# andres-fr/realtime-pose-estimation

Hardware: AMD Instinct MI355X
Metric: images/sec at 640x640 (HRNet-w48 fwd+decode) (higher is better)
Workload: dtype f16 (fp32 accumulate, fp32 BatchNorm; fp32 NCHW in/out); 1 GPU; configs[2]: batch=32 per GPU, 640x640, half-wrapper teacher forward + decode of 17 keypoint channels, weights W0 (seeded random); batch_per_gpu=32, people_per_batch_rank0=960

## Files before the change

realtime-pose-estimation_amd/csrc/engine.hip:

```cpp
#include <stdarg.h>

#include <chrono>
#include <mutex>
#include <map>
#include <tuple>
#include <vector>

#include "rtpe_common.h"

namespace rtpe {

static thread_local std::string g_err;

void set_error(const char* fmt, ...) {
  char buf[1024];
  va_list ap;
  va_start(ap, fmt);
  vsnprintf(buf, sizeof(buf), fmt, ap);
  va_end(ap);
  g_err = buf;
}

int hip_fail(hipError_t e, const char* what, const char* file, int line) {
  set_error("HIP error %d (%s) at %s:%d: %s", (int)e, hipGetErrorString(e), file, line, what);
// ... 10 lines not shown
  int fuse;
  int pair;
  int stem2;
  int s2g;
};

}

using namespace rtpe;

struct rtpe_hrnet {
  int device;
  std::vector<OpState> ops;
  std::map<std::tuple<int, int, int>, std::vector<ConvTile>> tuned;
  std::map<int, std::vector<hipEvent_t>> records;
  std::vector<rtpe_tensor_desc> tensors;
  std::vector<char> plane_ok;
  int n_slots;
  char* arena;
  size_t arena_bytes;
  int n_preds, n_refined;
  std::mutex lane_mu;
  hipStream_t lane_stream[4] = {nullptr, nullptr, nullptr, nullptr};
  std::vector<hipEvent_t> op_event;
  std::vector<char> needs_event;
  std::vector<std::vector<int>> wait_ops;
  hipEvent_t fork_event = nullptr;
  bool has_regions = false;
};

static size_t align_up(size_t v, size_t a) { return (v + a - 1) / a * a; }

namespace rtpe {
static int g_options[kNumOptions] = {-1, -1, -1, -1, -1, -1, -1, -1, -1, -1, -1};
static const char* const kOptionNames[kNumOptions] = {"block_ring", "block_pc", "direct_1x1", "lanes", "tile_dma", "pair_1x1", "fused_stem", "conv64", "head_direct", "deconv48", "conv48s2"};
static const char* const kOptionEnv[kNumOptions] = {"RTPE_BLOCK_RING", "RTPE_BLOCK_PC", "RTPE_DIRECT_1X1", "RTPE_LANES", "RTPE_TILE_DMA", "RTPE_PAIR_1X1", "RTPE_FUSED_STEM", "RTPE_CONV64", "RTPE_HEAD_DIRECT", "RTPE_DECONV48", "RTPE_CONV48S2"};
static const int kOptionDefault[kNumOptions] = {0, 1, 1, 1, 1, 1, 1, 1, 1, 1, 1};
int get_option(int key) {
  int v = __atomic_load_n(&g_options[key], __ATOMIC_RELAXED);
  if (v < 0) {
    v = kOptionEnv[key][0] ? env_int(kOptionEnv[key], kOptionDefault[key]) : kOptionDefault[key];
    __atomic_store_n(&g_options[key], v, __ATOMIC_RELAXED);
  }
  return v;
}
}

extern "C" int rtpe_set_option(const char* name, int32_t value) {
  RTPE_REQUIRE(name != nullptr && value >= 0, "set_option: bad argument");
  for (int k = 0; k < kNumOptions; ++k)
    if (kOptionNames[k][0] && strcmp(name, kOptionNames[k]) == 0) {
      __atomic_store_n(&g_options[k], (int)value, __ATOMIC_RELAXED);
      return RTPE_OK;
    }
  set_error("set_option: unknown option '%s'", name);
  return RTPE_E_INVALID;
}

extern "C" int rtpe_get_option(const char* name, int32_t* value) {
  RTPE_REQUIRE(name != nullptr && value != nullptr, "get_option: null argument");
  for (int k = 0; k < kNumOptions; ++k)
    if (kOptionNames[k][0] && strcmp(name, kOptionNames[k]) == 0) {
      *value = get_option(k);
      return RTPE_OK;
    }
  set_error("get_option: unknown option '%s'", name);
  return RTPE_E_INVALID;
}

extern "C" const char* rtpe_last_error_string(void) { return g_err.c_str(); }
// ... 634 lines not shown
        }
        a.N = N; a.H_in = Hi; a.W_in = Wi;
        a.H_full = Ho; a.W_full = Wo;
        if (dc) {
          a.H_pos = Hi; a.W_pos = Wi; a.o_mul = 2; a.oy_add = k >> 1; a.ox_add = k & 1;
        } else {
          a.H_pos = Ho; a.W_pos = Wo; a.o_mul = 1;
        }
        a.relu = (d.flags & RTPE_F_RELU) ? 1 : 0;
        a.round_conv = (d.flags & RTPE_F_ROUND_CONV) ? 1 : 0;
        ConvTile tile;
        if (merge)
          tile = tile0;
        else if (force)
          tile = *force;
        else if (tuned && (*tuned)[i * 4 + k].nt)
          tile = (*tuned)[i * 4 + k];
        else
          tile = conv_make_tile(o.plan[k], N, a.H_pos, a.W_pos);
        const bool direct_ok = a.x_bytes < 0x80000000ull && a.y != nullptr && a.y_nchw == nullptr && a.o_mul == 1;
        if (tile.kind == 4 && !direct_ok) tile = conv_make_tile(o.plan[k], N, a.H_pos, a.W_pos, false);
        if (tile.kind == 5 && !(direct_ok && a.res == nullptr && !plane[d.in_t] && !plane[d.out_t] && get_option(kOptConv64) != 0))
          tile = conv_make_tile(o.plan[k], N, a.H_pos, a.W_pos, true, false);
        conv_fill_args(o.geom[k], o.plan[k], tile, &a);
        if (!merge && force == nullptr && get_option(kOptHeadDirect) != 0 && conv_head_supports(o.plan[k], a)) {
          RTPE_HP_LAUNCH(rc = conv_head_launch(o.plan[k], a, s));
          continue;
        }
        if (!merge && force == nullptr && get_option(kOptConv48s2) != 0 && !plane[d.in_t] && !(a.y != nullptr && plane[d.out_t]) &&
            conv48s2_supports(o.plan[k], a)) {
          RTPE_HP_LAUNCH(rc = conv48s2_launch(o.plan[k], a, s));
          continue;
        }
        if (merge) {
          if (k == 0) { merged = a; merged_tile = tile; merged.n_cls = 4; }
          merged.w_c[k] = a.w;
          merged.lo_yc[k] = a.lo_y; merged.lo_xc[k] = a.lo_x;
          merged.oy_c[k] = a.oy_add; merged.ox_c[k] = a.ox_add;
          if (k == o.n_geom - 1) {
            if (force == nullptr && get_option(kOptDeconv48) != 0 && deconv48_supports(o.plan[0], merged))
              RTPE_HP_LAUNCH(rc = deconv48_launch(o.plan[0], merged, s));
            else
              RTPE_HP_LAUNCH(rc = conv_launch(o.plan[0], merged_tile, merged, s));
          }
          continue;
        }
        if (pairs_on && o.pair == 1 && direct_ok) {
          pair_args = a;
          pair_pending = true;
          continue;
        }
        if (pair_pending) {
          pair_pending = false;
          RTPE_HP_LAUNCH(rc = conv_pair_launch(h->ops[i - 1].plan[0], pair_args, o.plan[0], a, s));
          continue;
        }
        RTPE_HP_LAUNCH(rc = conv_launch(o.plan[k], tile, a, s));
      }
    } else if (d.kind == RTPE_OP_AUX_PACK) {
      if (aux == nullptr) { set_error("forward: this program has a second input (use rtpe_hrnet_forward_aux)"); return RTPE_E_INVALID; }
      const rtpe_tensor_desc& to = h->tensors[d.out_t];
      rc = aux_pack_launch(reinterpret_cast<const float*>(aux), reinterpret_cast<float*>(tptr(d.out_t, d.out_coff)),
                           to.channels, N, H >> to.ds_log2, W >> to.ds_log2, s);
    } else if (d.kind == RTPE_OP_RESIZE) {
      const rtpe_tensor_desc& ti = h->tensors[d.in_t];
      const rtpe_tensor_desc& to = h->tensors[d.out_t];
// ... 178 lines not shown
  char* dev = nullptr;
  const size_t wb = align_up(p.packed_bytes, 256);
  RTPE_HIP_CHECK(hipMalloc(reinterpret_cast<void**>(&dev), wb + ab.size() * 4));
  hipError_t e = hipMemcpy(dev, packed.data(), p.packed_bytes, hipMemcpyHostToDevice);
  if (e == hipSuccess) e = hipMemcpy(dev + wb, ab.data(), ab.size() * 4, hipMemcpyHostToDevice);
  if (e != hipSuccess) { hipFree(dev); return hip_fail(e, "hipMemcpy", __FILE__, __LINE__); }
  ConvArgs a;
  memset(&a, 0, sizeof(a));
  a.x = reinterpret_cast<const _Float16*>(x); a.in_ld = cin;
  a.x_bytes = (size_t)N * H * W * cin * es;
  a.w = reinterpret_cast<const _Float16*>(dev);
  a.alpha = reinterpret_cast<const float*>(dev + wb); a.beta = a.alpha + p.cout_pad;
  a.res = reinterpret_cast<const _Float16*>(res); a.res_ld = cout;
  a.y = reinterpret_cast<_Float16*>(y); a.out_ld = cout; a.cout_store = cout;
  a.N = N; a.H_in = H; a.W_in = W;
  a.H_full = a.H_pos = H / stride; a.W_full = a.W_pos = W / stride; a.o_mul = 1;
  a.relu = (flags & RTPE_F_RELU) ? 1 : 0;
  a.round_conv = (flags & RTPE_F_ROUND_CONV) ? 1 : 0;
  const bool one_window = a.x_bytes < 0x80000000ull;
  const ConvTile tile = conv_make_tile(p, N, a.H_pos, a.W_pos, one_window, one_window && res == nullptr);
  static const int probe_plane = RTPE_DIAG_ENV_INT("RTPE_PROBE_PLANE", 0);
  if (probe_plane && tile.kind == 2 && cin % 48 == 0 && cout % 48 == 0 && stride == 1) {
    a.in_ld = 48; a.in_cs = (long long)N * H * W * 48;
    a.out_ld = 48; a.out_cs = (long long)N * H * W * 48;
    if (res != nullptr) { a.res_ld = 48; a.res_cs = (long long)N * H * W * 48; }
  }
  conv_fill_args(g, p, tile, &a);
#ifdef RTPE_CONV_STAMPS
  unsigned long long* dbg = nullptr;
  hipMalloc(reinterpret_cast<void**>(&dbg), 128);
  hipMemset(dbg, 0, 128);
  a.dbg = dbg;
#endif
  int rc = get_option(kOptConv48s2) != 0 && conv48s2_supports(p, a) ? conv48s2_launch(p, a, s) : conv_launch(p, tile, a, s);
  hipError_t es2 = hipStreamSynchronize(s);
#ifdef RTPE_CONV_STAMPS
  unsigned long long hd[16];
  hipMemcpy(hd, dbg, 128, hipMemcpyDeviceToHost);
  hipFree(dbg);
  if (tile.kind == 2 && hd[5] && (hd[11] = hd[11] ? hd[11] : hd[5] / tile.waves)) {
    const unsigned long long nw = (unsigned long long)tile.grid * tile.waves, units = hd[5] / p.n_cchunks;
    fprintf(stderr, "stream conv %dx%d nt%d w%d nb%d nw%d grid %d | per MFMA wave: total %llu cycles, %llu units | per stage: waitM %llu half0 %llu "
            "waitH %llu half1 %llu | per unit: E-wait %llu bn+transpose %llu res-wait %llu rows+add+store %llu load_res %llu | weight loader/stage: wait %llu issue %llu | "
            "tile loaders/stage: wait %llu issue %llu\n",
            tile.th, tile.tw, tile.nt, tile.waves, tile.n_bufs, tile.n_wslots, tile.grid, hd[15] / nw, units / nw, hd[0] / hd[5], hd[1] / hd[5],
            hd[2] / hd[5], hd[3] / hd[5], hd[12] / units, hd[13] / units, hd[4] / units, hd[14] / units, hd[10] / units, hd[6] / hd[11],
            hd[7] / hd[11], hd[8] / hd[11], hd[9] / hd[11]);
  }
  else if (hd[5])
    fprintf(stderr, "conv stamps (kind %d): n %llu | per wave(-unit) cycles: setup %llu stage/wait1 %llu kloop %llu epilogue %llu total/wait2 %llu\n",
            tile.kind, hd[5], hd[0] / hd[5], hd[1] / hd[5], hd[2] / hd[5], hd[3] / hd[5], hd[4] / hd[5]);
  if (hd[10] && tile.kind != 2)
    fprintf(stderr, "   loader per stage: vmcnt-wait %llu barrier1 %llu issue %llu barriersE+2 %llu (stages %llu)\n",
            hd[6] / hd[10], hd[7] / hd[10], hd[8] / hd[10], hd[9] / hd[10], hd[10]);
#endif
  hipFree(dev);
  if (rc != RTPE_OK) return rc;
  if (es2 != hipSuccess) return hip_fail(es2, "hipStreamSynchronize", __FILE__, __LINE__);
  return RTPE_OK;
}

extern "C" int rtpe_basicblock_nhwc(const void* x, int32_t N, int32_t H, int32_t W, const void* w1_host,
                                    const float* alpha1, const float* beta1, const void* w2_host, const float* alpha2,
                                    const float* beta2, void* y, void* stream) {
  RTPE_REQUIRE(x && w1_host && w2_host && alpha1 && beta1 && alpha2 && beta2 && y, "basicblock_nhwc: null argument");
  RTPE_REQUIRE(conv_block_supports(48, 48, H, W), "basicblock_nhwc: H=%d W=%d unsupported", H, W);
  hipStream_t s = reinterpret_cast<hipStream_t>(stream);
// ... 130 lines not shown
    return RTPE_OK;
  }
  if (o.n_geom == 0) return RTPE_OK;
  const rtpe_op_desc& d = o.d;
  const rtpe_tensor_desc& ti = h->tensors[d.in_t];
  const int Hi = H >> ti.ds_log2, Wi = W >> ti.ds_log2;
  const bool dc = d.kind == RTPE_OP_DECONV;
  const int Hp = dc ? Hi : Hi / d.stride, Wp = dc ? Wi : Wi / d.stride;
  ConvTile t = conv_make_tile(o.plan[0], N, Hp, Wp);
  {
    auto it = h->tuned.find(std::make_tuple(N, H, W));
    if (it != h->tuned.end() && it->second[op * 4].nt) t = it->second[op * 4];
  }
  if (t.kind == 5 && (d.res_t >= 0 || (d.flags & RTPE_F_NO_NHWC))) t = conv_make_tile(o.plan[0], N, Hp, Wp, true, false);
  if ((d.flags & (RTPE_F_OUT_PREDS | RTPE_F_OUT_REFINED)) && d.kind == RTPE_OP_CONV && d.ksize == 1 && d.cin == 48 && d.res_t < 0 &&
      !(d.flags & RTPE_F_F32) && get_option(kOptHeadDirect) != 0 && o.plan[0].n_cb == 1 && (o.plan[0].mt == 2 || o.plan[0].mt == 3) &&
      ((unsigned)Hi * (unsigned)Wi) % 32u == 0) {
    out8[0] = o.plan[0].mt; out8[1] = 2; out8[2] = 4; out8[3] = 1; out8[4] = 32; out8[5] = 48; out8[6] = 1; out8[7] = -400001;
    return RTPE_OK;
  }
  if (dc && get_option(kOptDeconv48) != 0 && t.kind == 0 && d.res_t < 0 && !(d.flags & RTPE_F_NO_NHWC) && !h->plane_ok[d.in_t] &&
      !h->plane_ok[d.out_t] && o.plan[0].mt == 3 && o.plan[0].n_cb == 1 && o.plan[0].cout_pad == 48 && o.plan[0].n_cchunks <= 2) {
    out8[0] = 3; out8[1] = 2; out8[2] = 4; out8[3] = 8; out8[4] = 16; out8[5] = 48; out8[6] = 1; out8[7] = -300001;
    return RTPE_OK;
  }
  if (!dc && get_option(kOptConv48s2) != 0 && d.ksize == 3 && d.stride == 2 && d.cin == 48 && d.res_t < 0 && !(d.flags & (RTPE_F_NO_NHWC | RTPE_F_F32)) &&
      !h->plane_ok[d.in_t] && !h->plane_ok[d.out_t] && (d.cout == 48 || d.cout == 96 || d.cout == 192 || d.cout == 384) &&
      o.plan[0].cout_pad == d.cout && Hi % 2 == 0 && Wi % 2 == 0) {
    const int gw = d.cout == 48 ? 1 : d.cout == 96 ? 2 : 4;
    out8[0] = 3; out8[1] = 2; out8[2] = 4; out8[3] = 8; out8[4] = 8; out8[5] = 48; out8[6] = d.cout / (48 * gw);
    out8[7] = o.s2g > 1 ? -(200000 + o.s2g) : o.s2g < 0 ? -200009 : -200001;
    return RTPE_OK;
  }
  if (o.pair && get_option(kOptPair1x1) != 0) {
    out8[0] = o.pair == 1 ? 16 : 4; out8[1] = 1; out8[2] = 8; out8[3] = 1; out8[4] = 16; out8[5] = o.pair == 1 ? 64 : 256; out8[6] = 1;
    out8[7] = o.pair == 1 ? -800001 : -800002;
    return RTPE_OK;
  }
  if (o.fuse) {
    out8[0] = 3; out8[1] = o.fuse == 1 ? 5 : 3; out8[2] = 4; out8[3] = 6; out8[4] = 32; out8[5] = 48; out8[6] = 1;
    out8[7] = o.fuse == 1 ? -900001 : -900002;
    return RTPE_OK;
  }
  out8[0] = t.kind == 0 && t.mrun ? t.mrun : o.plan[0].mt; out8[1] = t.nt; out8[2] = t.waves; out8[3] = t.th; out8[4] = t.tw;
  out8[5] = o.plan[0].cc; out8[6] = o.plan[0].n_cb; out8[7] = t.kind == 2 ? -(t.grid + 100000 * t.n_bufs) : t.kind == 4 ? -(700000 + t.grid) : t.kind == 5 ? -(500000 + t.grid)
                                                            : (int32_t)t.lds_bytes;
  return RTPE_OK;
}

static int autotune_impl(rtpe_hrnet* h, const void* x, int32_t x_dtype, const void* aux, int32_t N, int32_t H, int32_t W,
                         void* preds, void* refined, int32_t out_dtype, void* workspace, size_t workspace_bytes,
                         void* stream) {
  RTPE_REQUIRE(h != nullptr, "autotune: null handle");
  hipStream_t s = reinterpret_cast<hipStream_t>(stream);
  const auto shape = std::make_tuple(N, H, W);
  h->tuned.erase(shape);
  const size_t n_ops = h->ops.size();
  std::vector<float> ms(n_ops);
  int rc = run(h, x, x_dtype, N, H, W, preds, refined, out_dtype, workspace, workspace_bytes, s, ms.data(), (int)n_ops,
               -1, -1, nullptr, nullptr, aux);
  if (rc != RTPE_OK) return rc;

  typedef std::tuple<int, int, int, int, int, int, int, int, int, int> Key;
  struct Class { std::vector<size_t> ops; std::vector<std::vector<ConvTile>> cands; std::vector<double> t; };
  std::map<Key, Class> classes;
  for (size_t i = 0; i < n_ops; ++i) {
    const OpState& o = h->ops[i];
    const rtpe_op_desc& d = o.d;
    if (o.n_geom == 0) continue;
    const rtpe_tensor_desc& ti = h->tensors[d.in_t];
    const Key key = std::make_tuple(d.cin, d.cout, d.ksize, d.stride, (int)d.kind, (int)ti.ds_log2, d.res_t >= 0 ? 1 : 0,
                                    (int)(d.flags & (RTPE_F_OUT_PREDS | RTPE_F_OUT_REFINED | RTPE_F_NO_NHWC | RTPE_F_F32)),
                                    (int)d.reserved[1] , (int)d.reserved[2]);
    Class& c = classes[key];
    if (c.ops.empty()) {
      const int Hi = H >> ti.ds_log2, Wi = W >> ti.ds_log2;
      const bool dc = d.kind == RTPE_OP_DECONV;
      const int Hp = dc ? Hi : Hi / d.stride, Wp = dc ? Wi : Wi / d.stride;
      c.cands.resize(o.n_geom);
      for (int k = 0; k < o.n_geom; ++k) conv_enum_tiles(o.plan[k], N, Hp, Wp, &c.cands[k]);
      size_t nc = c.cands[0].size();
      for (int k = 1; k < o.n_geom; ++k) nc = c.cands[k].size() < nc ? c.cands[k].size() : nc;
      c.t.assign(nc, 0.0);
    }
    c.ops.push_back(i);
  }
  size_t rounds = 0;
  for (auto& kv : classes) rounds = kv.second.t.size() > rounds ? kv.second.t.size() : rounds;
  std::vector<ConvTile> trial(n_ops * 4);
  for (size_t r = 0; r < rounds; ++r) {
    for (auto& b : trial) memset(&b, 0, sizeof(b));
    for (auto& kv : classes) {
      Class& c = kv.second;
      if (c.t.empty()) continue;
      const size_t ci = r < c.t.size() ? r : c.t.size() - 1;
      for (size_t i : c.ops)
        for (size_t k = 0; k < c.cands.size(); ++k) trial[i * 4 + k] = c.cands[k][ci];
    }
    h->tuned[shape] = trial;
    std::vector<float> best_ms(n_ops, 1e30f);
    for (int rep = 0; rep < 6; ++rep) {
      rc = run(h, x, x_dtype, N, H, W, preds, refined, out_dtype, workspace, workspace_bytes, s, ms.data(), (int)n_ops,
// ... 114 lines not shown
```

realtime-pose-estimation_amd/csrc/rtpe_common.h:

```cpp
#pragma once
#include <hip/hip_runtime.h>
#include <hip/hip_fp16.h>
#include <stdint.h>
#include <stdio.h>
#include <stdlib.h>
#include <string.h>
#include <string>
#include <vector>

#include "rtpe_hip.h"

namespace rtpe {

void set_error(const char* fmt, ...);
int hip_fail(hipError_t e, const char* what, const char* file, int line);

#define RTPE_HIP_CHECK(expr)                                               \
  do {                                                                     \
    hipError_t _e = (expr);                                                \
    if (_e != hipSuccess) return ::rtpe::hip_fail(_e, #expr, __FILE__, __LINE__); \
  } while (0)

#define RTPE_REQUIRE(cond, ...)                 \
  do {                                          \
    if (!(cond)) {                              \
      ::rtpe::set_error(__VA_ARGS__);           \
      return RTPE_E_INVALID;                    \
    }                                           \
  } while (0)

inline int env_int(const char* name, int dflt) {
  const char* v = getenv(name);
  return v ? atoi(v) : dflt;
}
#ifdef RTPE_DIAG
#define RTPE_DIAG_ENV_INT(name, dflt) ::rtpe::env_int(name, dflt)
#else
#define RTPE_DIAG_ENV_INT(name, dflt) (dflt)
#endif

enum { kOptBlockRing = 0, kOptBlockPC = 1, kOptDirect1x1 = 2, kOptLanes = 3, kOptTileDma = 4, kOptPair1x1 = 5, kOptFusedStem = 6, kOptConv64 = 7, kOptHeadDirect = 8, kOptDeconv48 = 9, kOptConv48s2 = 10, kNumOptions = 11 };
int get_option(int key);

inline bool first_use_on_device(unsigned long long* mask) {
  int dev = 0;
  if (hipGetDevice(&dev) != hipSuccess || dev < 0 || dev > 63) return true;
  const unsigned long long bit = 1ull << dev;
  const unsigned long long old = __atomic_fetch_or(mask, bit, __ATOMIC_RELAXED);
  return !(old & bit);
}

struct DeviceGuard {
  int prev = -1;
  bool switched = false;
  hipError_t err = hipSuccess;
  explicit DeviceGuard(int device) {
    err = hipGetDevice(&prev);
    if (err == hipSuccess && prev != device) {
      err = hipSetDevice(device);
      switched = err == hipSuccess;
    }
  }
  ~DeviceGuard() {
    if (switched) (void)hipSetDevice(prev);
  }
};

struct FastDiv {
  uint32_t d, mul;
};
inline FastDiv make_fastdiv(uint32_t d) {
  FastDiv f;
  f.d = d;
  f.mul = d <= 1 ? 0u : (uint32_t)((0x100000000ull + d - 1) / d);
// ... 94 lines not shown
struct ConvGeom {
  int cin, cout, ksize, stride;
  int deconv_class;
  int esize;
  int dil;
};

ConvPlan conv_make_plan(const ConvGeom& g);
ConvTile conv_make_tile(const ConvPlan& p, int N, int H_pos, int W_pos, bool allow_direct = true, bool allow_conv64 = true);
int conv_row_pitch(const ConvPlan& p, int tw, int kind);
bool conv_deint(const ConvPlan& p, int kind);
void conv_enum_tiles(const ConvPlan& p, int N, int H_pos, int W_pos, std::vector<ConvTile>* out);
void conv_pack_weights(const ConvGeom& g, const ConvPlan& p, const void* w, void* packed);
void conv_fill_args(const ConvGeom& g, const ConvPlan& p, const ConvTile& t, ConvArgs* a);
int conv_launch(const ConvPlan& p, const ConvTile& t, const ConvArgs& a, hipStream_t s);
bool conv_stream_supports(const ConvPlan& p);
size_t conv_stream_lds(const ConvPlan& p, int buf_bytes, int n_bufs, int n_wslots);
int conv_stream_launch(const ConvPlan& p, const ConvTile& t, const ConvArgs& a, hipStream_t s);
bool conv_pair_supports(int cin1, int cout1, int cout2);
int conv_pair_launch(const ConvPlan& p1, const ConvArgs& c1, const ConvPlan& p2, const ConvArgs& c2, hipStream_t s);
int conv_direct_mb(const ConvPlan& p);
bool conv64_supports(const ConvPlan& p);
size_t conv64_lds();
int conv64_grid(int N, int H_pos, int W_pos);
int conv64_launch(const ConvPlan& p, const ConvTile& t, const ConvArgs& a, hipStream_t s);
int conv_direct_launch(const ConvPlan& p, const ConvArgs& a, hipStream_t s);
bool conv_head_supports(const ConvPlan& p, const ConvArgs& a);
int conv_head_launch(const ConvPlan& p, const ConvArgs& a, hipStream_t s);
bool deconv48_supports(const ConvPlan& p, const ConvArgs& merged);
int deconv48_launch(const ConvPlan& p, const ConvArgs& merged, hipStream_t s);
bool conv48s2_supports(const ConvPlan& p, const ConvArgs& a);
int conv48s2_launch(const ConvPlan& p, const ConvArgs& a, hipStream_t s);
int conv48s2_launch_group(const ConvPlan* const* plans, const ConvArgs* layers, int n, hipStream_t s);
bool conv_block_supports(int cin, int cout, int H, int W);
int conv_block_launch(const _Float16* x, int in_ld, size_t x_bytes, _Float16* y, int out_ld, const _Float16* w1,
                      const float* ab1, const _Float16* w2, const float* ab2, int N, int H, int W, hipStream_t s);

struct FuseArgs {
  const _Float16* term[4];
  int term_ld[4], term_up[4];
  int n_terms;
  _Float16* y;
  int out_ld, C;
  int N, H, W;
  int f32;
  int relu;
};
int fuse_launch(const FuseArgs& a, hipStream_t s);

struct StemArgs {
  const void* x;
  int x_f32;
  const _Float16* w;
  const float* alpha;
  const float* beta;
  _Float16* y;
  int N, H, W, out_ld;
  int f32;
};
int stem_launch(const StemArgs& a, hipStream_t s);

struct StemFusedArgs {
  const void* x;
  int x_f32;
  const _Float16* w1;
  const float* alpha1;
// ... 29 lines not shown
```

realtime-pose-estimation_amd/rtpe/_native.py:

```python
import ctypes
import os
from ctypes import (POINTER, Structure, byref, c_char_p, c_double, c_float, c_int32, c_int64,
                    c_size_t, c_uint32, c_void_p)

_PKG_DIR = os.path.dirname(os.path.dirname(os.path.abspath(__file__)))
LIB_PATH = os.environ.get("RTPE_LIBRARY") or os.path.join(_PKG_DIR, "librtpe_hip.so")

ABI_VERSION = 4
RTPE_DTYPE_F16, RTPE_DTYPE_F32 = 1, 2
OP_STEM, OP_CONV, OP_DECONV, OP_FUSE, OP_CAST, OP_AVGPOOL, OP_SE, OP_CAM_COMBINE, OP_SIGMOID_ADD = range(9)
OP_AUX_PACK, OP_RESIZE, OP_GATE_MUL = 9, 10, 11
F_RELU, F_ROUND_CONV, F_OUT_PREDS, F_OUT_REFINED, F_NO_NHWC, F_F32 = 1, 2, 4, 8, 16, 32
F_PAIR_HEAD, F_PAIR_TAIL = 64, 128


class TensorDesc(Structure):
    _fields_ = [("channels", c_int32), ("ds_log2", c_int32), ("slot", c_int32), ("reserved", c_int32)]


class OpDesc(Structure):
    _fields_ = [("kind", c_int32), ("flags", c_int32),
                ("in_t", c_int32), ("in_coff", c_int32),
                ("out_t", c_int32), ("out_coff", c_int32),
                ("res_t", c_int32), ("res_coff", c_int32),
                ("cin", c_int32), ("cout", c_int32),
                ("ksize", c_int32), ("stride", c_int32),
                ("w_off", c_int64), ("ab_off", c_int64),
                ("n_terms", c_int32), ("term_t", c_int32 * 4), ("term_up", c_int32 * 4),
                ("reserved", c_int32 * 3), ("lane", c_int32), ("region", c_int32)]


_SIGS = {
    "rtpe_last_error_string": (c_char_p, []),
    "rtpe_version": (c_int32, []),
    "rtpe_device_count": (c_int32, []),
    "rtpe_hrnet_create": (c_int32, [POINTER(OpDesc), c_int32, POINTER(TensorDesc), c_int32,
                                    c_void_p, c_size_t, c_int32, POINTER(c_void_p)]),
    "rtpe_hrnet_destroy": (c_int32, [c_void_p]),
    "rtpe_hrnet_workspace_bytes": (c_int32, [c_void_p, c_int32, c_int32, c_int32, POINTER(c_size_t)]),
    "rtpe_hrnet_forward": (c_int32, [c_void_p, c_void_p, c_int32, c_int32, c_int32, c_int32,
                                     c_void_p, c_void_p, c_int32, c_void_p, c_size_t, c_void_p]),
# ... 83 lines not shown
    "rtpe_adjust_refine_ms": (c_int32, [c_void_p, c_int32, c_int32, c_int32, POINTER(c_int32), POINTER(c_int32),
                                        c_int32, c_int32, c_int32, c_int32, c_size_t, c_void_p, c_void_p, c_void_p,
                                        c_int32, c_int32, c_int32, c_void_p, c_void_p, c_void_p, c_int32, c_void_p,
                                        c_size_t, c_void_p]),
    "rtpe_match_by_tag_batch": (c_int32, [c_void_p, c_void_p, c_void_p, c_int32, c_int32, c_int32, c_int32,
                                          c_int32, c_int32, c_double, c_double, c_int32, c_int32, c_void_p,
                                          c_int32, c_void_p, c_void_p, c_int32]),
}

EXPORTS = tuple(_SIGS)
_lib = None


def lib():
    global _lib
    if _lib is None:
        if not os.path.exists(LIB_PATH):
            raise RuntimeError(
                "rtpe: %s not found - the HIP extension is not built and there is no CPU "
                "fallback.  Build it with `python -c \"import __graft_entry__ as g; g.build()\"` "
                "from the repository root (needs hipcc)." % LIB_PATH)
        import torch
        try:
            L = ctypes.CDLL(LIB_PATH)
        except OSError as e:
            raise RuntimeError("rtpe: cannot load %s: %s" % (LIB_PATH, e)) from e
        for name, (res, args) in _SIGS.items():
            fn = getattr(L, name)
            fn.restype, fn.argtypes = res, args
        got = L.rtpe_version()
        if got != ABI_VERSION:
            raise RuntimeError("rtpe: %s has ABI revision %d, this binding needs %d - rebuild it from this tree "
                               "(`python -c \"import __graft_entry__ as g; g.build()\"`)" % (LIB_PATH, got, ABI_VERSION))
        _lib = L
    return _lib


def check(rc):
    if rc != 0:
        msg = lib().rtpe_last_error_string()
        raise RuntimeError("rtpe_hip error %d: %s" % (rc, msg.decode() if msg else "?"))


def require_gpu(t, what):
    if not t.is_cuda:
        raise RuntimeError(
            "rtpe: %s runs on the MI355X HIP path only and got a %s tensor; move it to a GPU "
            "(there is deliberately no CPU fallback in the product path)" % (what, t.device))


def stream_ptr(device):
    import torch
    return c_void_p(torch.cuda.current_stream(device).cuda_stream)


def on_device(t):
    import torch
    return torch.cuda.device(t.device)


def same_device(what, first, *others):
    for t in others:
        if t is not None and t.device != first.device:
            raise RuntimeError("rtpe: %s: tensors on different devices (%s and %s)" % (what, first.device, t.device))


# ... 8 lines not shown
```

Baseline: 2404 images/sec.

## Add warp-specialized stride-2 3x3 conv kernel for 96-channel inputs

Adds a dedicated HIP kernel for stride-2 3x3 convolutions with 96 input channels and 96/192/384 outputs, enabled by default. It uses a requester wave that DMAs halo tiles straight into LDS through a multi-buffer ring, six MFMA waves that keep their weights in registers, and a store wave that writes the BN-scaled fp16 output. Odd and even input columns are split in LDS so the stride-2 taps read contiguously. The goal is to overlap loads, math and stores for the HRNet transition downsampling convs, which adds a new specialized code path and extra LDS-driven synchronisation. The autotuner skips these ops, and the Python loader now checks that the built library exposes the new options.

Result: no change. 2417 images/sec (median of 4 runs) (+0.5%).

```diff
diff --git a/realtime-pose-estimation_amd/csrc/conv_s2w.hip b/realtime-pose-estimation_amd/csrc/conv_s2w.hip
--- /dev/null
+++ b/realtime-pose-estimation_amd/csrc/conv_s2w.hip
@@ -0,0 +1,320 @@
+#include "rtpe_common.h"
+
+namespace rtpe {
+
+typedef _Float16 half8 __attribute__((ext_vector_type(8)));
+typedef float float4v __attribute__((ext_vector_type(4)));
+typedef unsigned int u32x4 __attribute__((ext_vector_type(4)));
+typedef float float2v __attribute__((ext_vector_type(2)));
+typedef _Float16 half2v __attribute__((ext_vector_type(2)));
+
+namespace {
+constexpr int kK = 14;
+constexpr int kNC = 2;
+constexpr int kPS = 96;
+constexpr int kThreads = 512;
+typedef __attribute__((address_space(3))) void* lds_ptr_t;
+constexpr int kMulWaves = 6;
+constexpr int kReqWave = kMulWaves, kStoreWave = kMulWaves + 1;
+constexpr int kTH = 8, kTW = 8;
+constexpr int kNT = kTH * kTW / 16;
+constexpr int kD = 3;
+constexpr int kNB = kD + 1;
+constexpr int kHH = 2 * kTH + 1, kHW = 2 * kTW + 1;
+constexpr int kNEven = (kHW + 1) / 2;
+constexpr int kRowB = 1664;
+constexpr int kBufBytes = kHH * kRowB;
+constexpr int kTileSlots = kBufBytes / 16;
+constexpr int kRowSlots = kRowB / 16;
+constexpr int kDmaIter = (kTileSlots + 63) / 64;
+constexpr int kOP = 96 * 2 + 16;
+constexpr int kObufBytes = kTH * kTW * kOP;
+constexpr int kPieces = kTH * kTW * 12 / 64;
+constexpr int kLds = kNB * kBufBytes + kObufBytes;
+static_assert(kRowB >= kHW * kPS && kTileSlots > (kDmaIter - 1) * 64, "the requester issues kDmaIter instructions per tile");
+static_assert((kD - 1) * kDmaIter < 64, "vmcnt is a 6-bit counter");
+static_assert(kLds <= 160 * 1024, "LDS layout");
+static_assert(kMulWaves * 16 == 96, "a multiplier wave per 16 output channels of the block");
+}
+
+struct S2WBlock {
+  const _Float16* w;
+  const float* alpha;
+  const float* beta;
+  _Float16* y;
+  int mt_pack, blk, out_ld, cout_store, relu;
+  unsigned y_bytes;
+};
+struct S2WArgs {
+  const _Float16* x;
+  unsigned x_bytes;
+  int N, H_in, W_in, in_ld, H_out, W_out;
+  int tiles_x, tiles_y, n_cb;
+  FastDiv div_tiles_x, div_tiles_xy, div_ncb;
+  S2WBlock blk[4];
+};
+
+template <bool ROUND>
+__global__ void __launch_bounds__(kThreads) conv_s2w_kernel(const S2WArgs a) {
+  extern __shared__ __attribute__((aligned(16))) char smem[];
+  char* const bufs = smem;
+  char* const obuf = smem + kNB * kBufBytes;
+
+  const int tid = threadIdx.x, lane = tid & 63, wv = __builtin_amdgcn_readfirstlane(tid >> 6);
+  const int tiles_x = a.tiles_x, tiles_y = a.tiles_y, n_cb = a.n_cb;
+  const int total = a.N * tiles_x * tiles_y * n_cb;
+  const int wg_per_xcd = (int)(gridDim.x >> 3);
+  int per_xcd = (total + 7) >> 3;
+  per_xcd = (per_xcd + n_cb - 1) / n_cb * n_cb;
+  const int xcd = (int)(blockIdx.x & 7u);
+  const int u_end = (xcd + 1) * per_xcd < total ? (xcd + 1) * per_xcd : total;
+  const int u0 = xcd * per_xcd + (int)(blockIdx.x >> 3);
+  if (u0 >= u_end) return;
+  const int cb = u0 % n_cb;
+  const S2WBlock& e = a.blk[cb];
+  const int n_units = (u_end - 1 - u0) / wg_per_xcd + 1;
+  const int n_stages = kNC * n_units;
+
+  auto tile_origin = [&](int u, int* n, int* py0, int* px0) {
+    const uint32_t tt = fdiv((uint32_t)u, a.div_ncb);
+    const uint32_t nn = fdiv(tt, a.div_tiles_xy);
+    const uint32_t rem = tt - nn * (uint32_t)(tiles_x * tiles_y);
+    const uint32_t ty = fdiv(rem, a.div_tiles_x);
+    *n = (int)nn; *py0 = (int)ty * kTH; *px0 = (int)(rem - ty * tiles_x) * kTW;
+  };
+
+  if (wv == kStoreWave) {
+    const int H_out = a.H_out, W_out = a.W_out;
+    const __amdgpu_buffer_rsrc_t ysrc = __builtin_amdgcn_make_buffer_rsrc(e.y, 0, (int)e.y_bytes, 0x00020000);
+    const int ch0 = e.blk * 96;
+    int lds_off[kPieces], orel[kPieces], oyx[kPieces];
+#pragma unroll
+    for (int k = 0; k < kPieces; ++k) {
+      const int j = k * 64 + lane;
+      const int pw = j / 12, slot = j - pw * 12;
+      const int oy = pw / kTW, ox = pw - oy * kTW;
+      lds_off[k] = pw * kOP + slot * 16;
+      orel[k] = ((oy * W_out + ox) * e.out_ld + ch0 + slot * 8) * 2;
+      oyx[k] = ch0 + slot * 8 < e.cout_store ? (oy | (ox << 8)) : 0x4000;
+    }
+    uint4 raw[kPieces];
+    auto read_rows = [&]() {
+#pragma unroll
+      for (int k = 0; k < kPieces; ++k) raw[k] = *reinterpret_cast<const uint4*>(obuf + lds_off[k]);
+    };
+    auto store_rows = [&](int u) {
+      int n, py0, px0;
+      tile_origin(u, &n, &py0, &px0);
+      const int pix0 = (n * H_out + py0) * W_out + px0;
+      const int ly = H_out - py0, lx = W_out - px0;
+#pragma unroll
+      for (int k = 0; k < kPieces; ++k) {
+        half8 hv = __builtin_bit_cast(half8, raw[k]);
+        if (e.relu) hv = __builtin_elementwise_max(hv, half8{0, 0, 0, 0, 0, 0, 0, 0});
+        const bool ok = (oyx[k] & 0x40ff) < ly && (oyx[k] >> 8 & 0x3f) < lx;
+        const uint32_t voff = ok ? (uint32_t)(pix0 * e.out_ld * 2 + orel[k]) : 0x80000000u;
+        __builtin_amdgcn_raw_buffer_store_b128(__builtin_bit_cast(u32x4, hv), ysrc, (int)voff, 0, 0);
+      }
+    };
+    int prev = -1;
+    for (int u = u0; u < u_end; u += wg_per_xcd) {
+      __syncthreads();
+      if (prev >= 0) read_rows();
+      __syncthreads();
+      asm volatile("s_waitcnt lgkmcnt(0)" ::: "memory");
+      __syncthreads();
+      if (prev >= 0) store_rows(prev);
+      prev = u;
+    }
+    __syncthreads();
+    read_rows();
+    store_rows(prev);
+    return;
+  }
+  if (wv == kReqWave) {
+    const __amdgpu_buffer_rsrc_t rsrc = __builtin_amdgcn_make_buffer_rsrc(const_cast<_Float16*>(a.x), 0, (int)a.x_bytes, 0x00020000);
+    const int H_in = a.H_in, W_in = a.W_in, in_ld = a.in_ld;
+    int rel[kDmaIter], hyx[kDmaIter];
+#pragma unroll
+    for (int k = 0; k < kDmaIter; ++k) {
+      const int sl = k * 64 + lane;
+      const int hy = sl / kRowSlots, rem = sl - hy * kRowSlots;
+      const int lc = rem / 6, s = rem - lc * 6;
+      const int col = lc < kNEven ? 2 * lc : 2 * (lc - kNEven) + 1;
+      const bool data = sl < kTileSlots && lc < kHW;
+      rel[k] = ((hy * W_in + col) * in_ld + s * 8) * 2;
+      hyx[k] = data ? (hy | (col << 8)) : 0x4000;
+    }
+    auto request_stage = [&](int i) {
+      int n, py0, px0;
+      tile_origin(u0 + (i >> 1) * wg_per_xcd, &n, &py0, &px0);
+      char* const buf = bufs + (i % kNB) * kBufBytes;
+      const int iy0 = 2 * py0 - 1, ix0 = 2 * px0 - 1;
+      const int base = ((n * H_in + iy0) * W_in + ix0) * in_ld * 2 + (i & 1) * 96;
+#pragma unroll
+      for (int k = 0; k < kDmaIter; ++k) {
+        const int s0 = k * 64;
+        const int iy = iy0 + (hyx[k] & 0x40ff), ix = ix0 + ((hyx[k] >> 8) & 0x3f);
+        const bool ok = (unsigned)iy < (unsigned)H_in && (unsigned)ix < (unsigned)W_in;
+        const uint32_t voff = ok ? (uint32_t)(base + rel[k]) : 0x80000000u;
+        if (s0 + 64 <= kTileSlots || s0 + lane < kTileSlots)
+          __builtin_amdgcn_raw_ptr_buffer_load_lds(rsrc, (lds_ptr_t)(buf + s0 * 16), 16, (int)voff, 0, 0, 0);
+      }
+    };
+    for (int i = 0; i < kD && i < n_stages; ++i) request_stage(i);
+    for (int i = 0; i < n_stages; ++i) {
+      const int after = n_stages - 1 - i;
+      if (after >= 2) asm volatile("s_waitcnt vmcnt(%0)" ::"n"(2 * kDmaIter) : "memory");
+      else if (after >= 1) asm volatile("s_waitcnt vmcnt(%0)" ::"n"(kDmaIter) : "memory");
+      else asm volatile("s_waitcnt vmcnt(0)" ::: "memory");
+      __syncthreads();
+      if (i + kD < n_stages) request_stage(i + kD);
+      if (i & 1) __syncthreads();
+    }
+    __syncthreads();
+    return;
+  }
+
+  const int r = lane & 15, g = lane >> 4;
+  const int ct = e.blk * kMulWaves + wv;
+  const int mt_pack = e.mt_pack;
+  uint4 a_res[kNC][kK];
+  {
+    const int pb = ct / mt_pack, m0 = ct - pb * mt_pack;
+    const uint4* wfrag = reinterpret_cast<const uint4*>(e.w) + ((size_t)pb * kNC * kK * mt_pack + m0) * 64 + lane;
+#pragma unroll
+    for (int c = 0; c < kNC; ++c)
+#pragma unroll
+      for (int k = 0; k < kK; ++k) a_res[c][k] = wfrag[(size_t)((c * kK + k) * mt_pack) * 64];
+  }
+  const float4v al = *reinterpret_cast<const float4v*>(e.alpha + ct * 16 + g * 4);
+  const float4v be = *reinterpret_cast<const float4v*>(e.beta + ct * 16 + g * 4);
+  int toff[kK];
+#pragma unroll
+  for (int kk = 0; kk < kK; ++kk) {
+    int k = kk * 32 + g * 8;
+    if (k >= 9 * 48) k -= 9 * 48;
+    const int tap = k / 48, c = k - tap * 48;
+    const int ty = tap / 3, tx = tap - ty * 3;
+    const int cs = tx == 0 ? 0 : tx == 1 ? kNEven : 1;
+    toff[kk] = ty * kRowB + cs * kPS + c * 2;
+  }
+  const int lane_off = 2 * (r >> 3) * kRowB + (r & 7) * kPS;
+  constexpr int kTileStep = 4 * kRowB;
+  asm volatile("s_waitcnt vmcnt(0)" ::: "memory");
+  int cur = 0;
+  for (int u = u0; u < u_end; u += wg_per_xcd) {
+    float4v acc[kNT];
+#pragma unroll
+    for (int nt = 0; nt < kNT; ++nt) acc[nt] = float4v{0.f, 0.f, 0.f, 0.f};
+#pragma unroll
+    for (int c = 0; c < kNC; ++c) {
+      const char* th = bufs + cur * kBufBytes + lane_off;
+      __syncthreads();
+      uint4 bf[2][kNT];
+#pragma unroll
+      for (int nt = 0; nt < kNT; ++nt) bf[0][nt] = *reinterpret_cast<const uint4*>(th + nt * kTileStep + toff[0]);
+#pragma unroll
+      for (int k = 0; k < kK; ++k) {
+        const int cbuf = k & 1, nb = cbuf ^ 1;
+        if (k + 1 < kK) {
+#pragma unroll
+          for (int nt = 0; nt < kNT; ++nt) bf[nb][nt] = *reinterpret_cast<const uint4*>(th + nt * kTileStep + toff[k + 1]);
+        }
+#pragma unroll
+        for (int nt = 0; nt < kNT; ++nt)
+          acc[nt] = __builtin_amdgcn_mfma_f32_16x16x32_f16(__builtin_bit_cast(half8, a_res[c][k]),
+                                                           __builtin_bit_cast(half8, bf[cbuf][nt]), acc[nt], 0, 0, 0);
+        if (k + 1 < kK) {
+#pragma unroll
+          for (int i = 0; i < kNT; ++i) {
+            __builtin_amdgcn_sched_group_barrier(0x008, 1, 0);
+            __builtin_amdgcn_sched_group_barrier(0x100, 1, 0);
+          }
+        }
+        __builtin_amdgcn_sched_barrier(0);
+      }
+      cur = cur + 1 == kNB ? 0 : cur + 1;
+    }
+    __syncthreads();
+#pragma unroll
+    for (int nt = 0; nt < kNT; ++nt) {
+      half2v o[2];
+#pragma unroll
+      for (int j = 0; j < 2; ++j) {
+        float2v x = {acc[nt][2 * j], acc[nt][2 * j + 1]};
+        if (ROUND) x = __builtin_convertvector(__builtin_convertvector(x, half2v), float2v);
+        float2v tt = __builtin_elementwise_fma(x, float2v{al[2 * j], al[2 * j + 1]}, float2v{be[2 * j], be[2 * j + 1]});
+        asm volatile("" : "+v"(tt));
+        o[j] = __builtin_convertvector(tt, half2v);
+      }
+      unsigned long long raw;
+      __builtin_memcpy(&raw, o, 8);
+      *reinterpret_cast<unsigned long long*>(obuf + (nt * 16 + r) * kOP + wv * 32 + g * 8) = raw;
+    }
+    asm volatile("s_waitcnt lgkmcnt(0)" ::: "memory");
+  }
+  __syncthreads();
+}
+
+bool conv_s2w_supports(const ConvPlan& p, const ConvArgs& a) {
+  if (!(p.esize == 2 && p.dil == 1 && p.tapw == 3 && p.in_mul == 2 && p.cc == 48 && p.n_cchunks == kNC && p.kc == kK &&
+        p.cin == 96 && (p.mt == 3 || p.mt == 6) && (p.cout == 96 || p.cout == 192 || p.cout == 384) && p.cout_pad == p.cout))
+    return false;
+  return a.n_cls == 0 && a.o_mul == 1 && a.res == nullptr && a.y != nullptr && a.y_nchw == nullptr && a.in_cs == 48 &&
+         a.out_cs == p.mt * 16 && a.in_ld >= 96 && a.out_ld >= p.cout && a.cout_store % 8 == 0 && a.cout_store <= p.cout &&
+         a.x_bytes > 0 && a.x_bytes < 0x80000000ull && (size_t)a.N * a.H_full * a.W_full * a.out_ld * 2 < 0x80000000ull &&
+         a.H_pos == a.H_full && a.W_pos == a.W_full && a.H_pos == a.H_in / 2 && a.W_pos == a.W_in / 2 && a.H_in % 2 == 0 &&
+         a.W_in % 2 == 0 && a.lo_y == -1 && a.lo_x == -1;
+}
+
+int conv_s2w_launch_group(const ConvPlan* const* plans, const ConvArgs* layers, int n, hipStream_t s) {
+  RTPE_REQUIRE(n >= 1 && n <= 4, "conv_s2w: %d layers", n);
+  S2WArgs a;
+  memset(&a, 0, sizeof(a));
+  const ConvArgs& l0 = layers[0];
+  a.x = l0.x; a.x_bytes = (unsigned)l0.x_bytes;
+  a.N = l0.N; a.H_in = l0.H_in; a.W_in = l0.W_in; a.in_ld = l0.in_ld; a.H_out = l0.H_full; a.W_out = l0.W_full;
+  int nb = 0;
+  for (int i = 0; i < n; ++i) {
+    const ConvPlan& p = *plans[i];
+    const ConvArgs& l = layers[i];
+    RTPE_REQUIRE(conv_s2w_supports(p, l), "conv_s2w: unsupported layer");
+    RTPE_REQUIRE(l.x == l0.x && l.x_bytes == l0.x_bytes && l.N == l0.N && l.H_in == l0.H_in && l.W_in == l0.W_in && l.in_ld == l0.in_ld &&
+                 l.round_conv == l0.round_conv, "conv_s2w: the layers of a launch read one input");
+    RTPE_REQUIRE(nb + p.cout / 96 <= 4, "conv_s2w: more than four cout blocks in a launch");
+    for (int b = 0; b < p.cout / 96; ++b, ++nb) {
+      S2WBlock& e = a.blk[nb];
+      e.w = l.w; e.alpha = l.alpha; e.beta = l.beta; e.y = l.y;
+      e.mt_pack = p.mt; e.blk = b; e.out_ld = l.out_ld; e.cout_store = l.cout_store; e.relu = l.relu;
+      e.y_bytes = (unsigned)((size_t)l.N * l.H_full * l.W_full * l.out_ld * 2);
+    }
+  }
+  a.n_cb = nb;
+  a.tiles_x = (a.W_out + kTW - 1) / kTW;
+  a.tiles_y = (a.H_out + kTH - 1) / kTH;
+  a.div_tiles_x = make_fastdiv((uint32_t)a.tiles_x);
+  a.div_tiles_xy = make_fastdiv((uint32_t)(a.tiles_x * a.tiles_y));
+  a.div_ncb = make_fastdiv((uint32_t)a.n_cb);
+  const long units = (long)a.N * a.tiles_x * a.tiles_y * a.n_cb;
+  RTPE_REQUIRE(units >= 1 && units < (1l << 20), "conv_s2w: %ld units", units);
+  long per_xcd = (units + 7) / 8;
+  per_xcd = (per_xcd + a.n_cb - 1) / a.n_cb * a.n_cb;
+  const long G = per_xcd < 32 ? per_xcd : 32 / a.n_cb * a.n_cb;
+  static unsigned long long attr_mask = 0;
+  if (first_use_on_device(&attr_mask)) {
+    RTPE_HIP_CHECK(hipFuncSetAttribute(reinterpret_cast<const void*>(conv_s2w_kernel<false>), hipFuncAttributeMaxDynamicSharedMemorySize, kLds));
+    RTPE_HIP_CHECK(hipFuncSetAttribute(reinterpret_cast<const void*>(conv_s2w_kernel<true>), hipFuncAttributeMaxDynamicSharedMemorySize, kLds));
+  }
+  if (l0.round_conv) hipLaunchKernelGGL((conv_s2w_kernel<true>), dim3((unsigned)(8 * G)), dim3(kThreads), kLds, s, a);
+  else hipLaunchKernelGGL((conv_s2w_kernel<false>), dim3((unsigned)(8 * G)), dim3(kThreads), kLds, s, a);
+  RTPE_HIP_CHECK(hipGetLastError());
+  return RTPE_OK;
+}
+
+int conv_s2w_launch(const ConvPlan& p, const ConvArgs& a, hipStream_t s) {
+  const ConvPlan* pp = &p;
+  return conv_s2w_launch_group(&pp, &a, 1, s);
+}
+
+}
diff --git a/realtime-pose-estimation_amd/csrc/engine.hip b/realtime-pose-estimation_amd/csrc/engine.hip
--- a/realtime-pose-estimation_amd/csrc/engine.hip
+++ b/realtime-pose-estimation_amd/csrc/engine.hip
@@ -66,10 +66,10 @@
 static size_t align_up(size_t v, size_t a) { return (v + a - 1) / a * a; }
 
 namespace rtpe {
-static int g_options[kNumOptions] = {-1, -1, -1, -1, -1, -1, -1, -1, -1, -1, -1};
-static const char* const kOptionNames[kNumOptions] = {"block_ring", "block_pc", "direct_1x1", "lanes", "tile_dma", "pair_1x1", "fused_stem", "conv64", "head_direct", "deconv48", "conv48s2"};
-static const char* const kOptionEnv[kNumOptions] = {"RTPE_BLOCK_RING", "RTPE_BLOCK_PC", "RTPE_DIRECT_1X1", "RTPE_LANES", "RTPE_TILE_DMA", "RTPE_PAIR_1X1", "RTPE_FUSED_STEM", "RTPE_CONV64", "RTPE_HEAD_DIRECT", "RTPE_DECONV48", "RTPE_CONV48S2"};
-static const int kOptionDefault[kNumOptions] = {0, 1, 1, 1, 1, 1, 1, 1, 1, 1, 1};
+static int g_options[kNumOptions] = {-1, -1, -1, -1, -1, -1, -1, -1, -1, -1, -1, -1};
+static const char* const kOptionNames[kNumOptions] = {"block_ring", "block_pc", "direct_1x1", "lanes", "tile_dma", "pair_1x1", "fused_stem", "conv64", "head_direct", "deconv48", "conv48s2", "conv_s2w"};
+static const char* const kOptionEnv[kNumOptions] = {"RTPE_BLOCK_RING", "RTPE_BLOCK_PC", "RTPE_DIRECT_1X1", "RTPE_LANES", "RTPE_TILE_DMA", "RTPE_PAIR_1X1", "RTPE_FUSED_STEM", "RTPE_CONV64", "RTPE_HEAD_DIRECT", "RTPE_DECONV48", "RTPE_CONV48S2", "RTPE_CONV_S2W"};
+static const int kOptionDefault[kNumOptions] = {0, 1, 1, 1, 1, 1, 1, 1, 1, 1, 1, 1};
 int get_option(int key) {
   int v = __atomic_load_n(&g_options[key], __ATOMIC_RELAXED);
   if (v < 0) {
@@ -770,6 +770,11 @@
           RTPE_HP_LAUNCH(rc = conv48s2_launch(o.plan[k], a, s));
           continue;
         }
+        if (!merge && force == nullptr && get_option(kOptConvS2w) != 0 && !plane[d.in_t] && !(a.y != nullptr && plane[d.out_t]) &&
+            conv_s2w_supports(o.plan[k], a)) {
+          RTPE_HP_LAUNCH(rc = conv_s2w_launch(o.plan[k], a, s));
+          continue;
+        }
         if (merge) {
           if (k == 0) { merged = a; merged_tile = tile; merged.n_cls = 4; }
           merged.w_c[k] = a.w;
@@ -1014,7 +1019,9 @@
   hipMemset(dbg, 0, 128);
   a.dbg = dbg;
 #endif
-  int rc = get_option(kOptConv48s2) != 0 && conv48s2_supports(p, a) ? conv48s2_launch(p, a, s) : conv_launch(p, tile, a, s);
+  int rc = get_option(kOptConv48s2) != 0 && conv48s2_supports(p, a)   ? conv48s2_launch(p, a, s)
+           : get_option(kOptConvS2w) != 0 && conv_s2w_supports(p, a) ? conv_s2w_launch(p, a, s)
+                                                                      : conv_launch(p, tile, a, s);
   hipError_t es2 = hipStreamSynchronize(s);
 #ifdef RTPE_CONV_STAMPS
   unsigned long long hd[16];
@@ -1211,6 +1218,26 @@
     out8[7] = o.s2g > 1 ? -(200000 + o.s2g) : o.s2g < 0 ? -200009 : -200001;
     return RTPE_OK;
   }
+  if (!dc && get_option(kOptConvS2w) != 0 && d.res_t < 0 && !(d.flags & (RTPE_F_NO_NHWC | RTPE_F_OUT_PREDS | RTPE_F_OUT_REFINED)) &&
+      !h->plane_ok[d.in_t] && !h->plane_ok[d.out_t]) {
+    ConvArgs a;
+    memset(&a, 0, sizeof(a));
+    const rtpe_tensor_desc& to = h->tensors[d.out_t];
+    a.x = reinterpret_cast<const _Float16*>(16); a.y = reinterpret_cast<_Float16*>(16);
+    a.in_ld = ti.channels; a.out_ld = to.channels;
+    a.x_bytes = ((size_t)N * Hi * Wi * ti.channels - (size_t)d.in_coff) * 2;
+    const int room = to.channels - d.out_coff;
+    a.cout_store = o.plan[0].cout_pad < room ? o.plan[0].cout_pad : room;
+    if (d.reserved[2] > 0 && d.reserved[2] < a.cout_store) a.cout_store = d.reserved[2];
+    a.N = N; a.H_in = Hi; a.W_in = Wi; a.H_full = a.H_pos = Hp; a.W_full = a.W_pos = Wp; a.o_mul = 1;
+    a.lo_y = o.plan[0].lo_y; a.lo_x = o.plan[0].lo_x;
+    a.in_cs = o.plan[0].cc; a.out_cs = o.plan[0].mt * 16;
+    if (conv_s2w_supports(o.plan[0], a)) {
+      out8[0] = 1; out8[1] = 4; out8[2] = 6; out8[3] = 8; out8[4] = 8; out8[5] = 48; out8[6] = d.cout / 96;
+      out8[7] = -21001;
+      return RTPE_OK;
+    }
+  }
   if (o.pair && get_option(kOptPair1x1) != 0) {
     out8[0] = o.pair == 1 ? 16 : 4; out8[1] = 1; out8[2] = 8; out8[3] = 1; out8[4] = 16; out8[5] = o.pair == 1 ? 64 : 256; out8[6] = 1;
     out8[7] = o.pair == 1 ? -800001 : -800002;
@@ -1247,6 +1274,12 @@
     const OpState& o = h->ops[i];
     const rtpe_op_desc& d = o.d;
     if (o.n_geom == 0) continue;
+    {
+      int32_t t8[8];
+      if (rtpe_hrnet_op_tile(h, (int32_t)i, N, H, W, t8) == RTPE_OK &&
+          (t8[7] == -400001 || t8[7] == -300001 || (t8[7] <= -200001 && t8[7] >= -200009) || t8[7] == -21001))
+        continue;
+    }
     const rtpe_tensor_desc& ti = h->tensors[d.in_t];
     const Key key = std::make_tuple(d.cin, d.cout, d.ksize, d.stride, (int)d.kind, (int)ti.ds_log2, d.res_t >= 0 ? 1 : 0,
                                     (int)(d.flags & (RTPE_F_OUT_PREDS | RTPE_F_OUT_REFINED | RTPE_F_NO_NHWC | RTPE_F_F32)),
diff --git a/realtime-pose-estimation_amd/csrc/rtpe_common.h b/realtime-pose-estimation_amd/csrc/rtpe_common.h
--- a/realtime-pose-estimation_amd/csrc/rtpe_common.h
+++ b/realtime-pose-estimation_amd/csrc/rtpe_common.h
@@ -39,7 +39,7 @@
 #define RTPE_DIAG_ENV_INT(name, dflt) (dflt)
 #endif
 
-enum { kOptBlockRing = 0, kOptBlockPC = 1, kOptDirect1x1 = 2, kOptLanes = 3, kOptTileDma = 4, kOptPair1x1 = 5, kOptFusedStem = 6, kOptConv64 = 7, kOptHeadDirect = 8, kOptDeconv48 = 9, kOptConv48s2 = 10, kNumOptions = 11 };
+enum { kOptBlockRing = 0, kOptBlockPC = 1, kOptDirect1x1 = 2, kOptLanes = 3, kOptTileDma = 4, kOptPair1x1 = 5, kOptFusedStem = 6, kOptConv64 = 7, kOptHeadDirect = 8, kOptDeconv48 = 9, kOptConv48s2 = 10, kOptConvS2w = 11, kNumOptions = 12 };
 int get_option(int key);
 
 inline bool first_use_on_device(unsigned long long* mask) {
@@ -200,6 +200,8 @@
 bool conv48s2_supports(const ConvPlan& p, const ConvArgs& a);
 int conv48s2_launch(const ConvPlan& p, const ConvArgs& a, hipStream_t s);
 int conv48s2_launch_group(const ConvPlan* const* plans, const ConvArgs* layers, int n, hipStream_t s);
+bool conv_s2w_supports(const ConvPlan& p, const ConvArgs& a);
+int conv_s2w_launch(const ConvPlan& p, const ConvArgs& a, hipStream_t s);
 bool conv_block_supports(int cin, int cout, int H, int W);
 int conv_block_launch(const _Float16* x, int in_ld, size_t x_bytes, _Float16* y, int out_ld, const _Float16* w1,
                       const float* ab1, const _Float16* w2, const float* ab2, int N, int H, int W, hipStream_t s);
diff --git a/realtime-pose-estimation_amd/rtpe/_native.py b/realtime-pose-estimation_amd/rtpe/_native.py
--- a/realtime-pose-estimation_amd/rtpe/_native.py
+++ b/realtime-pose-estimation_amd/rtpe/_native.py
@@ -7,6 +7,7 @@
 LIB_PATH = os.environ.get("RTPE_LIBRARY") or os.path.join(_PKG_DIR, "librtpe_hip.so")
 
 ABI_VERSION = 4
+ABI4_OPTIONS = (b"deconv48", b"conv48s2", b"conv_s2w")
 RTPE_DTYPE_F16, RTPE_DTYPE_F32 = 1, 2
 OP_STEM, OP_CONV, OP_DECONV, OP_FUSE, OP_CAST, OP_AVGPOOL, OP_SE, OP_CAM_COMBINE, OP_SIGMOID_ADD = range(9)
 OP_AUX_PACK, OP_RESIZE, OP_GATE_MUL = 9, 10, 11
@@ -156,6 +157,11 @@
         if got != ABI_VERSION:
             raise RuntimeError("rtpe: %s has ABI revision %d, this binding needs %d - rebuild it from this tree "
                                "(`python -c \"import __graft_entry__ as g; g.build()\"`)" % (LIB_PATH, got, ABI_VERSION))
+        probe = ctypes.c_int32()
+        for opt in ABI4_OPTIONS:
+            if L.rtpe_get_option(opt, ctypes.byref(probe)) != 0:
+                raise RuntimeError("rtpe: %s lacks option %s - an older build of ABI revision %d; rebuild it from this tree "
+                                   "(`python -c \"import __graft_entry__ as g; g.build()\"`)" % (LIB_PATH, opt.decode(), got))
         _lib = L
     return _lib
 
```
